# HJakeCunningham/ASVGP

Hardware: AMD Instinct MI355X
Metric: Mpoints/s per ELBO+grad step, N=10M 1D Matern-3/2 M=2048 (higher is better)
Workload: dtype f64

## Files before the change

asvgp_amd/_lib.py:

```python
import ctypes
import os

import torch

HERE = os.path.dirname(os.path.abspath(__file__))
LIB_PATH = os.path.join(HERE, "libasvgp_hip.so")

_c = ctypes
_P, _I, _L, _D, _Z = _c.c_void_p, _c.c_int, _c.c_int64, _c.c_double, _c.c_size_t

SIGNATURES = {
    "asvgp_version": (_I, []),
    "asvgp_last_error_string": (_c.c_char_p, []),
    "asvgp_status_name": (_c.c_char_p, [_I]),
    "asvgp_phi_workspace_bytes": (_Z, [_L, _I, _L]),
    "asvgp_create": (_I, [_c.POINTER(_P)]),
    "asvgp_destroy": (_I, [_P]),
    "asvgp_phi_accumulate_1d": (_I, [_P, _P, _P, _L, _L, _P, _L, _D, _I, _L, _P, _P, _Z, _P]),
    "asvgp_phi_weighted_workspace_bytes": (_Z, [_L, _I, _L]),
    "asvgp_phi_accumulate_1d_weighted": (_I, [_P, _P, _P, _P, _L, _L, _P, _L, _D, _I, _L, _P, _P, _P, _Z, _P]),
    "asvgp_set_weight_sums": (_I, [_P, _D, _D, _D]),
    "asvgp_phi_accumulate_kron2d_weighted": (_I, [_P, _P, _P, _L, _P, _L, _D, _L, _P, _L, _D, _L, _I, _P, _P, _P]),
    "asvgp_phi_accumulate_kron2d_sorted_weighted": (_I, [_P, _P, _P, _L, _P, _P, _L, _D, _L, _P, _L, _D, _L, _I, _P, _P, _P]),
    "asvgp_set_phi_algorithm": (_I, [_P, _I]),
    "asvgp_phi_last_algorithm": (_I, [_P]),
    "asvgp_set_phi_input_order": (_I, [_P, _I]),
    "asvgp_phi_last_input_order": (_I, [_P]),
    "asvgp_stream_probe": (_I, [_P, _P, _L, _P, _P]),
    "asvgp_debug_reload_env": (_I, []),
    "asvgp_set_deferred_forward_pass": (_I, [_P, _I]),
    "asvgp_prior_publish": (_I, [_P]),
    "asvgp_host_mantissa_bits": (_I, []),
    "asvgp_prior_interior_kuu_host": (_I, [_P, _I, _L, _I, _P, _P, _c.POINTER(_L), _c.POINTER(_L), _P]),
    "asvgp_result_mirror": (_I, [_P, _I, _c.POINTER(_P)]),
    "asvgp_result_mirror_read": (_I, [_P, _c.c_uint64, _P, _D]),
    "asvgp_elbo_grad_ahead_1d": (_I, [_P, _P, _P, _I, _L, _L, _I, _L, _P, _P, _P, _Z, _P]),
    "asvgp_elbo_publish_theta": (_I, [_P, _D, _D, _D]),
    "asvgp_elbo_grad_host_1d": (_I, [_P, _P, _P, _I, _D, _D, _D, _L, _L, _I, _L, _P, _P, _P, _Z, _P, _P, _D]),
    "asvgp_result_mirror_pending": (_c.c_uint64, [_P]),
    "asvgp_set_phi_workgroups": (_I, [_P, _I]),
    "asvgp_set_phi_deferred_reduce": (_I, [_P, _I]),
    "asvgp_phi_reduce_1d": (_I, [_P, _P]),
    "asvgp_phi_index_1d": (_I, [_P, _L, _P, _L, _D, _P, _P]),
    "asvgp_phi_evaluate_1d": (_I, [_P, _L, _P, _L, _D, _I, _I, _P, _P, _P]),
    "asvgp_matern_coeffs": (_I, [_I, _D, _D, _c.POINTER(_D), _c.POINTER(_D), _c.POINTER(_I)]),
    "asvgp_kuu_assemble": (_I, [_P, _I, _c.POINTER(_D), _c.POINTER(_D), _L, _I, _P, _P, _P]),
    "asvgp_cholesky_band": (_I, [_P, _P, _L, _I, _P, _P]),
    "asvgp_inverse_from_cholesky_band": (_I, [_P, _P, _L, _I, _P]),
    "asvgp_solve_triang_mat": (_I, [_P, _P, _P, _L, _I, _L, _I, _P]),
    "asvgp_product_band_band": (_I, [_P, _P, _P, _L, _I, _I, _I, _I, _I, _I, _P]),
    "asvgp_transpose_band": (_I, [_P, _P, _L, _I, _I, _P]),
    "asvgp_symmetrise_band": (_I, [_P, _P, _L, _I, _P]),
    "asvgp_unpack_banded_matrix_to_dense": (_I, [_P, _P, _L, _I, _I, _P]),
    "asvgp_pack_dense_matrix_to_banded": (_I, [_P, _P, _L, _I, _I, _P]),
    "asvgp_band_trace_sym": (_I, [_P, _P, _L, _I, _P, _P]),
    "asvgp_cholesky_band_vjp": (_I, [_P, _P, _P, _P, _L, _I, _P]),
    "asvgp_inverse_from_cholesky_band_vjp": (_I, [_P, _P, _P, _P, _P, _L, _I, _P]),
    "asvgp_band_outer_product": (_I, [_P, _P, _L, _L, _I, _D, _P, _P]),
    "asvgp_elbo_workspace_bytes": (_Z, [_L, _I, _L]),
    "asvgp_set_band_algorithm": (_I, [_P, _I]),
    "asvgp_prior_plan_1d": (_I, [_P, _P, _I, _L, _I, _c.POINTER(_I)]),
    "asvgp_prior_table_doubles": (_Z, [_P, _I, _L, _I]),
    "asvgp_prior_forward_host": (_I, [_P, _I, _L, _I, _P, _P, _P, _Z, _P]),
    "asvgp_set_prior_forward": (_I, [_P, _I]),
    "asvgp_prior_forward_device": (_I, [_P, _P, _P, _P, _Z, _P]),
# ... 109 lines not shown
        import numpy as np
        coef = np.ascontiguousarray(coef, dtype=np.float64)
        dcoef = np.ascontiguousarray(dcoef, dtype=np.float64)
        tab = np.zeros(int(n_doubles), dtype=np.float64)
        check(self._lib.asvgp_prior_forward_device(self.ptr, coef.ctypes.data, dcoef.ctypes.data, tab.ctypes.data, tab.size, stream_ptr()),
              "prior_forward_device")
        return tab

    def set_band_algorithm(self, algo):
        check(self._lib.asvgp_set_band_algorithm(self.ptr, int(algo)), "set_band_algorithm")
        self.band_algorithm = int(algo)

    def set_phi_algorithm(self, algo):
        check(self._lib.asvgp_set_phi_algorithm(self.ptr, int(algo)), "set_phi_algorithm")

    def set_weight_sums(self, n_pos, sum_w, sum_log_w):
        if n_pos is None:
            n_pos, sum_w, sum_log_w = -1.0, 0.0, 0.0
        check(self._lib.asvgp_set_weight_sums(self.ptr, float(n_pos), float(sum_w), float(sum_log_w)), "set_weight_sums")

    def phi_last_algorithm(self):
        return int(self._lib.asvgp_phi_last_algorithm(self.ptr))

    def set_phi_input_order(self, order):
        check(self._lib.asvgp_set_phi_input_order(self.ptr, int(order)), "set_phi_input_order")

    def phi_last_input_order(self):
        return int(self._lib.asvgp_phi_last_input_order(self.ptr))

    def result_mirror(self, enable=True):
        import numpy as np
        ptr = _P()
        check(self._lib.asvgp_result_mirror(self.ptr, int(bool(enable)), ctypes.byref(ptr)), "result_mirror")
        if not enable or not ptr.value:
            self._mirror = None
            return None
        self._mirror = np.ctypeslib.as_array(ctypes.cast(ptr, ctypes.POINTER(_D)), shape=(16,))
        return self._mirror

    def set_deferred_forward_pass(self, on):
        check(self._lib.asvgp_set_deferred_forward_pass(self.ptr, int(on)), "set_deferred_forward_pass")

    def publish_forward(self):
        self._lib.asvgp_prior_publish(self.ptr)

    def result_mirror_pending(self):
# ... 79 lines not shown
```

asvgp_amd/csrc/handle.hip:

```cpp
#include <sched.h>
#include <stdlib.h>
#include <string.h>
#include <time.h>

#include <condition_variable>
#include <mutex>
#include <thread>
#include <vector>

#include "handle.hpp"

namespace asvgp {

static DebugEnv g_dbg;
static std::once_flag g_dbg_once;
static void debug_env_load() {
  g_dbg.no_assembly = getenv("ASVGP_DEBUG_NO_ASSEMBLY") ? 1 : 0;
  g_dbg.chain_stamps = getenv("ASVGP_CHAIN_STAMPS") ? 1 : 0;
  g_dbg.spin_limit = getenv("ASVGP_SPIN_LIMIT") ? atol(getenv("ASVGP_SPIN_LIMIT")) : (1L << 25);
  g_dbg.host_times = getenv("ASVGP_HOST_TIMES") ? 1 : 0;
  g_dbg.plan_first = getenv("ASVGP_PLAN_FIRST") ? 1 : 0;
  g_dbg.bcr_stamps = getenv("ASVGP_BCR_STAMPS") ? atoi(getenv("ASVGP_BCR_STAMPS")) : 0;
  g_dbg.no_split = getenv("ASVGP_NO_SPLIT") ? atoi(getenv("ASVGP_NO_SPLIT")) : 0;
}
const DebugEnv& debug_env() {
  std::call_once(g_dbg_once, debug_env_load);
  return g_dbg;
}

static Handle* g_default = nullptr;
static std::mutex g_default_mu;

Handle* as_handle(asvgp_handle_t h) {
  if (h) return reinterpret_cast<Handle*>(h);
  std::lock_guard<std::mutex> lk(g_default_mu);
  if (!g_default) {
    g_default = new Handle;
    (void)hipGetDevice(&g_default->device);
  }
  return g_default;
}

static void handle_quiesce(Handle* h) {
  if (h->ahead.valid) (void)elbo_publish_theta(h, 1.0, 1.0, 1.0, true);
  handle_publish_forward(h);
  bool need_sync = false;
// ... 164 lines not shown
  return ASVGP_OK;
}

extern "C" int asvgp_create(asvgp_handle_t* out) {
  if (!out) { set_error("asvgp_create: bad argument"); return ASVGP_ERR_BAD_ARG; }
  Handle* h = new Handle;
  if (hipGetDevice(&h->device) != hipSuccess) { delete h; set_error("asvgp_create: no HIP device"); return ASVGP_ERR_HIP; }
  *out = reinterpret_cast<asvgp_handle_t>(h);
  return ASVGP_OK;
}

extern "C" int asvgp_destroy(asvgp_handle_t handle) {
  if (!handle) return ASVGP_OK;
  Handle* h = reinterpret_cast<Handle*>(handle);
  if (h->magic != 0x41535647u) { set_error("asvgp_destroy: not a handle"); return ASVGP_ERR_BAD_ARG; }
  worker_stop(h);
  plan_release(h);
  if (h->mirror_host) (void)hipHostFree(h->mirror_host);
  if (h->evK) (void)hipEventDestroy(h->evK);
  if (h->evP) (void)hipEventDestroy(h->evP);
  if (h->prof_made)
    for (int i = 0; i < PROF_RING; ++i) { (void)hipEventDestroy(h->prof_ev[i][0]); (void)hipEventDestroy(h->prof_ev[i][1]); }
  if (h->order_dev) { (void)hipFree(h->order_dev); h->order_dev = nullptr; }
  if (h->box_host) { (void)hipHostFree(h->box_host); h->box_host = nullptr; h->box_dev = nullptr; }
  h->magic = 0;
  delete h;
  return ASVGP_OK;
}

extern "C" int asvgp_set_phi_algorithm(asvgp_handle_t handle, int algo) {
  if (algo != 0 && algo != 1 && algo != 3 && algo != 5 && algo != 6) {
    set_error("set_phi_algorithm: 0 auto (6 where it applies, else 5, else 3), 1 fp64 LDS-atomic band scatter, 3 fixed-point band scatter, 5 fixed-point centred-moment scatter, 6 tile sort + register moments");
    return ASVGP_ERR_BAD_ARG;
  }
  as_handle(handle)->phi_algo = algo;
  return ASVGP_OK;
}

extern "C" int asvgp_set_phi_input_order(asvgp_handle_t handle, int order) {
  if (order < 0 || order > 2) { set_error("set_phi_input_order: 0 probe once per (x, N), 1 unsorted, 2 time series"); return ASVGP_ERR_BAD_ARG; }
  Handle* h = as_handle(handle);
  h->phi_order = order;
  h->n_order_seen = 0;
  return ASVGP_OK;
}

// ... 191 lines not shown
```

asvgp_amd/csrc/handle.hpp:

```cpp
#pragma once
#include "asvgp_common.hpp"
#include "prior_plan.hpp"

namespace asvgp {

constexpr int PROF_RING = 1024;
constexpr int TAB_SLOTS = 16;

struct Handle {
  unsigned magic = 0x41535647u;
  int device = 0;
  int phi_algo = 0, phi_blocks = 0;
  int phi_last = 0;
  bool phi_defer = false;
  struct PendingReduce { const double* partials; int G, M, K; double* stats; bool valid; const int* ranges; } pend = {nullptr, 0, 0, 0, nullptr, false, nullptr};
  int band_algo = 0;
  bool sync_on = false;
  hipEvent_t evK = nullptr, evP = nullptr;
  bool prof_on = false, prof_made = false;
  int prof_every = 1;
  long prof_calls = 0, prof_n = 0;
  hipEvent_t prof_ev[PROF_RING][2];
  PriorPlan* plan = nullptr;
  int* node_rec_dev = nullptr;
// ... 12 lines not shown
  void* worker_park = nullptr;
  int wstate = 0;
  struct PendingForward { bool valid; double coef[ASVGP_MAX_KUU_TERMS], dcoef[ASVGP_MAX_KUU_TERMS]; double* tab; int slot; unsigned long long seq; } fwd = {false, {0}, {0}, nullptr, 0, 0};
  bool prior_forward_gpu = false;
  int* dd_img_i = nullptr;
  int dd_n_img = 0;
  double* dd_img_d = nullptr;
  double* dd_tab = nullptr;
  hipStream_t dd_stream = nullptr;
  unsigned long long* dd_ready = nullptr;
  double* mirror_host = nullptr;
  double* mirror_dev = nullptr;
  unsigned long long mirror_seq = 0;
  unsigned long long mirror_pending = 0;
  struct MeshSeen { const double* ptr; long n; int regular; double step, first, last; };
  MeshSeen mesh_seen[8];
  int n_mesh_seen = 0;
  int phi_order = 0;
  struct OrderSeen { const double* ptr; long n; int series; };
  OrderSeen order_seen[8];
  int n_order_seen = 0;
  int* order_dev = nullptr;
  int phi_last_series = 0;
  bool ahead_req = false;
  void* box_host = nullptr;
  void* box_dev = nullptr;
  struct PendingAhead { bool valid; int slot; unsigned long long seq; double* tab; int kind; double N, Nw, cw; } ahead = {false, 0, 0, nullptr, 0, 0.0, 0.0, 0.0};
  bool w_set = false;
  double w_npos = 0.0, w_sum = 0.0, w_sumlog = 0.0;
};
constexpr size_t BOX_BYTES = 4096;

struct DebugEnv { int no_assembly; int chain_stamps; long spin_limit; int host_times; int plan_first; int bcr_stamps; int no_split; };
const DebugEnv& debug_env();

Handle* as_handle(asvgp_handle_t h);

bool handle_mesh_is_linspace(Handle* h, const double* mesh_dev, long n_mesh, hipStream_t st, double* step_out, double* first_out, double* last_out);

int handle_flush_phi_reduce(Handle* h, const double* stats, hipStream_t st);

void handle_publish_forward(Handle* h);
void handle_post_forward(Handle* h);

int handle_prior_dd_prepare(Handle* h);
void handle_prior_dd_release(Handle* h);
int handle_prior_dd_forward(Handle* h, const double* coef, const double* dcoef, int slot, hipStream_t st, double** tab_out, unsigned long long* stamps = nullptr,
                            unsigned long long seq = 0, const unsigned long long** ready_out = nullptr);

int elbo_publish_theta(Handle* h, double v, double l, double s, bool withdraw);

double* handle_table_acquire(Handle* h, unsigned long long* seq_out, int* slot_out);

}
```

asvgp_amd/csrc/phi_pass.hip:

```cpp
#include <stdlib.h>

#include "handle.hpp"

namespace asvgp {

constexpr int PHI_THREADS = 1024;
constexpr int PHI_CH = 32;
constexpr int PHI_MAX_BLOCKS = 256;
constexpr size_t PHI_LDS_BUDGET = 160 * 1024 - 512;

template <int K> struct FxTab {
  int g[K + 1];
  constexpr FxTab() : g{} {
    double cf[K + 1][K + 1] = {};
    for (int i = 0; i <= K; ++i)
      for (int p = 0; p <= K; ++p) cf[i][p] = piece_coef<K, 0>(i, p);
    for (int d = 0; d <= K; ++d) {
      double mx = 0.0;
      for (int i = 0; i + d <= K; ++i)
        for (int q = 0; q <= 32; ++q) {
          const double t = q / 32.0;
          double a = cf[i][K], b = cf[i + d][K];
          for (int p = K - 1; p >= 0; --p) { a = a * t + cf[i][p]; b = b * t + cf[i + d][p]; }
          if (a * b > mx) mx = a * b;
// ... 658 lines not shown
  if (lane == 0 && good) atomicAdd(count, 1);
}

static bool handle_phi_is_series(Handle* h, const double* x, long N, double m0, double inv_delta, long n_mesh, hipStream_t st) {
  if (h->phi_order == 1) return false;
  if (h->phi_order == 2) return true;
  for (int i = 0; i < h->n_order_seen; ++i)
    if (h->order_seen[i].ptr == x && h->order_seen[i].n == N) return h->order_seen[i].series != 0;
  int series = 0;
  const int nprobe = 512;
  if (N >= 128L * nprobe) {
    if (!h->order_dev && hipMalloc(&h->order_dev, sizeof(int)) != hipSuccess) h->order_dev = nullptr;
    int cnt = 0;
    if (h->order_dev && hipMemsetAsync(h->order_dev, 0, sizeof(int), st) == hipSuccess) {
      hipLaunchKernelGGL(phi_order_probe_kernel, dim3(nprobe), dim3(64), 0, st, x, N, N / nprobe, nprobe, m0, inv_delta, (int)n_mesh, h->order_dev);
      if (hipMemcpyAsync(&cnt, h->order_dev, sizeof(int), hipMemcpyDeviceToHost, st) == hipSuccess && hipStreamSynchronize(st) == hipSuccess)
        series = cnt * 10 >= nprobe * 9 ? 1 : 0;
    }
  }
  if (h->n_order_seen < 8) h->order_seen[h->n_order_seen++] = Handle::OrderSeen{x, N, series};
  return series != 0;
}

template <int K, int TP, int TS>
static int launch_phi_sort_as(Handle* h, const double* x, const double* y, long N, const double* mesh, long n_mesh, double delta,
                              long M, double* stats, double* ws, hipStream_t st, double step, double m0, double m_last, double margin) {
  size_t lds_bytes = ps_lds_bytes<K, TP, TS>();
  if (ps_epilogue_bytes<K>() > lds_bytes) lds_bytes = ps_epilogue_bytes<K>();
  if (lds_bytes > 160 * 1024) return 1;
  long nblk = (N + TP * PS_THREADS - 1) / (TP * PS_THREADS);
  const long gmax = (h->phi_blocks > 0 && h->phi_blocks < PHI_MAX_BLOCKS) ? h->phi_blocks : PHI_MAX_BLOCKS;
  const int G = (int)(nblk < 1 ? 1 : (nblk > gmax ? gmax : nblk));
  long ppb = (N + G - 1) / G;
  ppb = TS ? ((ppb + 127) & ~127L) : ((ppb + 1) & ~1L);
  if (ppb > 0x3fffffffL) return 1;
  PsArgs a;
  a.x = x; a.y = y; a.N = N; a.mesh_g = mesh; a.n_mesh = (int)n_mesh; a.inv_delta = 1.0 / delta; a.M = (int)M;
  a.m0 = m0; a.m_last = m_last; a.step = step; a.smax_fast = 0.5 - margin;
  a.partials = ws; a.ppb = ppb; a.zero_ptr = stats; a.zero_n = (K + 2) * M + 1; a.stamps = nullptr; a.stamps_wave = 0;
  a.ranges = reinterpret_cast<int*>(ws + (size_t)PHI_MAX_BLOCKS * ((size_t)(K + 2) * M + 1));
  auto kern = phi_sort_kernel<K, TP, 0, 1, TS>;
  hipError_t e = hipFuncSetAttribute(reinterpret_cast<const void*>(kern), hipFuncAttributeMaxDynamicSharedMemorySize, (int)lds_bytes);
  if (e != hipSuccess) { set_error("hipFuncSetAttribute(%zu B LDS): %s", lds_bytes, hipGetErrorString(e)); return ASVGP_ERR_LDS_CAPACITY; }
  const bool prof = h->prof_on && h->prof_n < PROF_RING && (h->prof_calls++ % h->prof_every == 0);
  if (prof) (void)hipEventRecord(h->prof_ev[h->prof_n][0], st);
  hipLaunchKernelGGL(kern, dim3((unsigned)G), dim3(PS_THREADS), lds_bytes, st, a);
  if (prof) { (void)hipEventRecord(h->prof_ev[h->prof_n][1], st); ++h->prof_n; }
  h->phi_last_series = TS;
  const int E1 = (int)((K + 2) * M + 1);
  const int gsplit = G >= 64 ? 16 : (G >= 8 ? 4 : 1);
  if (h->phi_defer) {
    h->pend = Handle::PendingReduce{a.partials, G, (int)M, K, stats, true, a.ranges};
    return check_launch("phi_accumulate_1d (tile sort, reduce deferred)");
  }
  hipLaunchKernelGGL(phi_reduce_kernel, dim3((E1 + 255) / 256, gsplit), dim3(256), 0, st, a.partials, G, (int)M, K, 0, M, 1L, 0, 1, stats, (const int*)a.ranges);
  return check_launch("phi_accumulate_1d (tile sort)");
}

template <int K>
static int launch_phi_sort(Handle* h, const double* x, const double* y, long N, long D, const double* mesh, long n_mesh, double delta,
                           long M, double* stats, double* ws, hipStream_t st) {
  if (D != 1 || N < 2 || M > PS_NCELL || ((reinterpret_cast<uintptr_t>(x) | reinterpret_cast<uintptr_t>(y)) & 15) != 0) return 1;
  double step = 0.0, m0 = 0.0, m_last = 0.0;
  if (!handle_mesh_is_linspace(h, mesh, n_mesh, st, &step, &m0, &m_last)) return 1;
  const double amax = fabs(m0) > fabs(m_last) ? fabs(m0) : fabs(m_last);
  const double margin = 16.0 * 2.220446049250313e-16 * amax / delta + 1e-12;
  if (!(margin < 0.125)) return 1;
  constexpr int TP = ps_tile_points<K>();
  constexpr int TPS = TP < 4 ? TP : 4;
  if (handle_phi_is_series(h, x, N, m0, 1.0 / delta, n_mesh, st)) {
    const int rc = launch_phi_sort_as<K, TPS, 1>(h, x, y, N, mesh, n_mesh, delta, M, stats, ws, st, step, m0, m_last, margin);
// ... 141 lines not shown
  long ppb = ((long)N + G - 1) / G;
  ppb = (ppb + 1) & ~1L;
  hipLaunchKernelGGL(stream_probe_kernel, dim3(G), dim3(1024), 0, as_stream(stream), x, y, (long)N, ppb, sink);
  return check_launch("stream_probe");
}

namespace asvgp {
int handle_flush_phi_reduce(Handle* h, const double* stats, hipStream_t st) {
  if (!h->pend.valid) return ASVGP_OK;
  if (stats && stats != h->pend.stats) return ASVGP_OK;
  const Handle::PendingReduce p = h->pend;
  h->pend.valid = false;
  const int E1 = (p.K + 2) * p.M + 1;
  const int gsplit = p.G >= 64 ? 16 : (p.G >= 8 ? 4 : 1);
  hipLaunchKernelGGL(phi_reduce_kernel, dim3((E1 + 255) / 256, gsplit), dim3(256), 0, st, p.partials, p.G, p.M, p.K, 0, (long)p.M, 1L, 0, 1, p.stats, p.ranges);
  return check_launch("phi_reduce_1d");
}
}

extern "C" int asvgp_phi_reduce_1d(asvgp_handle_t handle, asvgp_stream_t stream) {
  return handle_flush_phi_reduce(as_handle(handle), nullptr, as_stream(stream));
}

extern "C" int asvgp_phi_index_1d(const double* x, int64_t N, const double* mesh, int64_t n_mesh, double delta,
                                  int64_t* idx, asvgp_stream_t stream) {
  if (!x || !mesh || !idx || N < 0 || n_mesh < 2 || !(delta > 0.0)) { set_error("phi_index_1d: bad argument"); return ASVGP_ERR_BAD_ARG; }
  if (N == 0) return ASVGP_OK;
  hipLaunchKernelGGL(phi_index_kernel, dim3((unsigned)((N + 255) / 256)), dim3(256), 0, as_stream(stream), x, (long)N,
                     mesh, (int)n_mesh, 1.0 / delta, reinterpret_cast<long long*>(idx));
  return check_launch("phi_index_1d");
}

template <int K>
static int launch_eval(const double* x, long N, const double* mesh, int n_mesh, double delta, int deriv,
                       long long* rows, double* data, hipStream_t st) {
  dim3 g((unsigned)((N + 255) / 256)), b(256);
  double id = 1.0 / delta;
  switch (deriv) {
    case 0: hipLaunchKernelGGL((phi_evaluate_kernel<K, 0>), g, b, 0, st, x, N, mesh, n_mesh, id, rows, data); break;
    case 1: hipLaunchKernelGGL((phi_evaluate_kernel<K, (K >= 1 ? 1 : 0)>), g, b, 0, st, x, N, mesh, n_mesh, id, rows, data); break;
    case 2: hipLaunchKernelGGL((phi_evaluate_kernel<K, (K >= 2 ? 2 : 0)>), g, b, 0, st, x, N, mesh, n_mesh, id, rows, data); break;
    default: hipLaunchKernelGGL((phi_evaluate_kernel<K, (K >= 3 ? 3 : 0)>), g, b, 0, st, x, N, mesh, n_mesh, id, rows, data); break;
  }
  return check_launch("phi_evaluate_1d");
}

// ... 122 lines not shown
```

asvgp_amd/csrc/phi_sort.hpp:

```cpp
#pragma once

namespace asvgp {

constexpr int PS_THREADS = 1024;
constexpr int PS_NCELL = 2 * PS_THREADS;
constexpr int PS_HEAVY = 48;
constexpr int PS_HROUND = 16;
constexpr int PS_HLIST = 8192 / (PS_HEAVY + 1) + 1;

struct PsArgs {
  const double* x; const double* y; long N;
  const double* mesh_g; int n_mesh; double inv_delta; int M;
  double m0, m_last;
  double step;
  double smax_fast;
  double* partials;
  long ppb;
  double* zero_ptr; long zero_n;
  unsigned long long* stamps;
  int stamps_wave;
  int* ranges;
};

template <int K> constexpr int ps_tile_points() { return K <= 3 ? 8 : (K == 4 ? 6 : (K == 5 ? 4 : 2)); }
#ifndef PS_GW
#define PS_GW 4
#endif
constexpr int PS_TS_SLOTS = 256;
template <int K> constexpr size_t ps_ts_bytes() { return (size_t)PS_TS_SLOTS * (3 * K + 2) * 8 + (size_t)2 * PS_TS_SLOTS * 4; }
template <int K, int TP, int TS = 0> constexpr size_t ps_lds_bytes() {
  return (size_t)(TP * PS_THREADS + 1) * 16 + (size_t)3 * PS_NCELL * 4 + 64 * 4 + 64 * 8 +
         (size_t)PS_HROUND * (3 * K + 1) * 8 + (size_t)PS_HLIST * 12 + (TS ? ps_ts_bytes<K>() : 0);
}
template <int K> constexpr size_t ps_epilogue_bytes() {
  int all = (K + 1) * (K + 2) / 2, lo = (K + 1) + K, hi = all - lo;
  int planes = K <= 4 ? all : (lo > hi ? lo : hi);
  if (planes < 2 * (K + 1)) planes = 2 * (K + 1);
  return (size_t)planes * (PS_THREADS + K) * 8;
}

__device__ __forceinline__ void ps_lds_barrier() { asm volatile("s_waitcnt lgkmcnt(0)\n\ts_barrier" ::: "memory"); }

template <int CTRL, int ROW_MASK>
__device__ __forceinline__ unsigned ps_dpp_add_u32(unsigned v) {
  return v + (unsigned)__builtin_amdgcn_update_dpp(0, (int)v, CTRL, ROW_MASK, 0xf, true);
// ... 86 lines not shown
  for (int q = 0; q <= K; ++q) T2[q] = 0.0;
  for (unsigned sl = (unsigned)first; sl < nsl; sl += (unsigned)stride) {
    const unsigned j = sl * 64 + lane;
    if (j < hn) {
      const double2 pt = buf[ho + j];
      ps_acc<K>(pt.x, pt.y, S2, T2);
    }
  }
  if constexpr (NS <= 8) {
    int idx;
    const double t = ps_reduce_scatter8<NS>(S2, lane, idx);
    if (lane < 8 && idx < NS) lds_add(slot + idx, t);
  } else {
#pragma unroll
    for (int q = 0; q < NS; ++q) { const double t = wave_sum_dpp(S2[q]); if (lane == 0) lds_add(slot + q, t); }
  }
  __builtin_amdgcn_sched_barrier(0);
  {
    int idx;
    const double t = ps_reduce_scatter8<K + 1>(T2, lane, idx);
    if (lane < 8 && idx <= K) lds_add(slot + NS + idx, t);
  }
  __builtin_amdgcn_sched_barrier(0);
}

template <int K, int TP, int ABL = 0, int PF = 0, int TS = 0>
__global__ __launch_bounds__(PS_THREADS) void phi_sort_kernel(PsArgs a) {
  extern __shared__ double lds[];
  static_assert(TP % 2 == 0 && TP * PS_THREADS <= 8192, "tile: rank field is 13 bits");
  constexpr int T = TP * PS_THREADS;
  constexpr int NS = 2 * K;
  double2* buf = reinterpret_cast<double2*>(lds);
  unsigned* cnt = reinterpret_cast<unsigned*>(buf + T + 1);
  unsigned* off = cnt + 2 * PS_NCELL;
  unsigned* wtot = off + PS_NCELL;
  double* scratch = reinterpret_cast<double*>(wtot + 64);
  constexpr int NSTAT = 3 * K + 1;
  double* hacc = scratch + 64;
  unsigned* hlist = reinterpret_cast<unsigned*>(hacc + PS_HROUND * NSTAT);
  unsigned* nheavy_p = wtot + 32;
  constexpr int TSW = NSTAT + 1;
  double* tstab = reinterpret_cast<double*>(hlist + 3 * PS_HLIST);
  int* tskey = reinterpret_cast<int*>(tstab + PS_TS_SLOTS * TSW);
  int* tslist = tskey + PS_TS_SLOTS;
  unsigned* ts_ctl = wtot + 40;
  if (a.zero_ptr) for (long e = (long)blockIdx.x * blockDim.x + threadIdx.x; e < a.zero_n; e += (long)gridDim.x * blockDim.x) a.zero_ptr[e] = 0.0;
// ... 472 lines not shown
  if (a.ranges) {
    const unsigned mn = n0A ? (unsigned)tid : (n0B ? (unsigned)(tid + PS_THREADS) : 0x7fffffu);
    const unsigned mx = n0B ? (unsigned)(tid + PS_THREADS) + 1u : (n0A ? (unsigned)tid + 1u : 0u);
    const unsigned wmn = ps_wave_min_u32(mn), wmx = ps_wave_max_u32(mx);
    if (lane == 0) { wtot[wv] = wmn; wtot[16 + wv] = wmx; }
    __syncthreads();
    const unsigned bmn = ps_wave_min_u32(wtot[lane & 15]), bmx = ps_wave_max_u32(wtot[16 + (lane & 15)]);
    col_lo = bmx ? (int)bmn : 1;
    col_hi = bmx ? (int)bmx - 1 + K : 0;
    if (col_hi > M - 1) col_hi = M - 1;
    if (tid == 0) { a.ranges[2 * blockIdx.x] = col_lo; a.ranges[2 * blockIdx.x + 1] = col_hi; }
    __syncthreads();
  }
  if constexpr (ABL == 5) {
    double keep = (double)(n0A + n0B);
#pragma unroll
    for (int p = 0; p < NS; ++p) keep += SA[p] + SB[p];
#pragma unroll
    for (int p = 0; p <= K; ++p) keep += TA[p] + TB[p];
    out[tid] = keep;
  } else if constexpr (ABL == 0 || ABL == 9) {
    constexpr int IW = PS_THREADS + K;
    double* img = lds;
    auto q_planes = [&](const double (&S)[NS], unsigned n0, int slot, int d0, int d1) __attribute__((always_inline)) {
      const double s0v = (double)n0;
      int pid = 0;
      if (!__any(n0 != 0u)) {
#pragma unroll
        for (int d = d0; d < d1; ++d)
#pragma unroll
          for (int i = 0; i + d <= K; ++i) img[(pid++) * IW + slot] = 0.0;
        return;
      }
#pragma unroll
      for (int d = d0; d < d1; ++d) {
#pragma unroll
        for (int i = 0; i + d <= K; ++i) {
          const int j = i + d, mi = K - j, mj = K - i;
          if (mi < i) continue;
          double e = MomCoef<K>::tab.pair[i][j][0] * s0v, o = 0.0;
#pragma unroll
          for (int p = 2; p <= NS; p += 2) e = fma(MomCoef<K>::tab.pair[i][j][p], S[p - 1], e);
          if (mi != i) {
#pragma unroll
            for (int p = 1; p <= NS; p += 2) o = fma(MomCoef<K>::tab.pair[i][j][p], S[p - 1], o);
            img[(pid + mi) * IW + slot] = e - o;
// ... 24 lines not shown
#pragma unroll
      for (int rnd = 0; rnd < (DSPLIT <= K ? 2 : 1); ++rnd) {
        const int d0 = rnd == 0 ? 0 : DSPLIT, d1 = rnd == 0 ? DSPLIT : K + 1;
        if (half == 0) q_planes(SA, n0A, K + tid, d0, d1); else q_planes(SB, n0B, K + tid, d0, d1);
        if (tid >= PS_THREADS - K) {
          const int hs = tid - (PS_THREADS - K);
          if (half == 0) {
            int np = 0;
#pragma unroll
            for (int d = d0; d < d1; ++d) np += K + 1 - d;
            for (int pl = 0; pl < np; ++pl) img[pl * IW + hs] = 0.0;
          } else {
            q_planes(SA, n0A, hs, d0, d1);
          }
        }
        ps_lds_barrier();
        if (j < M && j >= col_lo && j <= col_hi) {
          int pid = 0;
#pragma unroll
          for (int d = d0; d < d1; ++d) {
            double v = 0.0;
#pragma unroll
            for (int jj = d; jj <= K; ++jj) v += img[(pid + jj - d) * IW + tid + jj];
            __builtin_nontemporal_store((j + d < M) ? v : 0.0, out + (size_t)d * M + j);
            pid += K + 1 - d;
          }
        }
        ps_lds_barrier();
      }
    }
    r_planes(TA, K + tid, 0);
    r_planes(TB, K + tid, K + 1);
    if (tid >= PS_THREADS - K) {
      const int hs = tid - (PS_THREADS - K);
#pragma unroll
      for (int i = 0; i <= K; ++i) img[i * IW + hs] = 0.0;
      r_planes(TA, hs, K + 1);
    }
    ps_lds_barrier();
#pragma unroll
    for (int half = 0; half < 2; ++half) {
      const int j = half * PS_THREADS + tid;
      if (j < M && j >= col_lo && j <= col_hi) {
        double r = 0.0;
#pragma unroll
        for (int i = 0; i <= K; ++i) r += img[(half * (K + 1) + i) * IW + tid + i];
        __builtin_nontemporal_store(r, out + (size_t)(K + 1) * M + j);
      }
    }
    if (tid == 0) out[(size_t)(K + 2) * M] = (badf > 0.0) ? __builtin_nan("") : tot;
  } else {
    if (tid == 0) out[0] = tot + badf;
  }
  stamp(4);
  if constexpr (ABL == 9) {
    if (tid == (int)(a.stamps_wave * 64) && a.stamps)
      for (int i = 0; i < 8; ++i) a.stamps[(size_t)blockIdx.x * 8 + i] = ph[i];
  }
}

}
```

include/asvgp_hip.h:

```cpp
#ifndef ASVGP_HIP_H
#define ASVGP_HIP_H

#include <stddef.h>
#include <stdint.h>

#ifdef __cplusplus
extern "C" {
#endif

typedef void* asvgp_stream_t;
typedef struct asvgp_handle_s* asvgp_handle_t;

typedef enum {
  ASVGP_OK = 0,
  ASVGP_ERR_BAD_ARG = -1,
  ASVGP_ERR_UNSUPPORTED = -2,
  ASVGP_ERR_LDS_CAPACITY = -3,
  ASVGP_ERR_WORKSPACE = -4,
  ASVGP_ERR_HIP = -5
} asvgp_status;

enum { ASVGP_MATERN12 = 0, ASVGP_MATERN32 = 1, ASVGP_MATERN52 = 2 };
enum { ASVGP_MAX_ORDER = 6, ASVGP_MAX_BANDWIDTH = 8, ASVGP_MAX_KUU_TERMS = 9 };

// ... 13 lines not shown
int asvgp_prior_interior_kuu_host(const double* static_bands_host, int n_terms, int64_t M, int k, const double* coef_host,
                                  double* kuu_diag8, int64_t* lo, int64_t* hi, double* bnd256);
int asvgp_host_mantissa_bits(void);
int asvgp_debug_reload_env(void);
int asvgp_set_deferred_forward_pass(asvgp_handle_t handle, int on);
int asvgp_prior_publish(asvgp_handle_t handle);
int asvgp_result_mirror(asvgp_handle_t handle, int enable, const double** host_ptr);
uint64_t asvgp_result_mirror_pending(asvgp_handle_t handle);
int asvgp_result_mirror_read(asvgp_handle_t handle, uint64_t token, double* result10, double timeout_seconds);
int asvgp_elbo_grad_ahead_1d(asvgp_handle_t handle, const double* stats, const double* static_bands, int kind, int64_t N, int64_t M, int k,
                             int64_t D, double* out, int* info, void* workspace, size_t workspace_bytes, asvgp_stream_t stream);
int asvgp_elbo_publish_theta(asvgp_handle_t handle, double variance, double lengthscale, double noise_variance);
int asvgp_elbo_grad_host_1d(asvgp_handle_t handle, const double* stats, const double* static_bands, int kind, double variance,
                            double lengthscale, double noise_variance, int64_t N, int64_t M, int k, int64_t D,
                            double* out, int* info, void* workspace, size_t workspace_bytes, asvgp_stream_t stream,
                            double* result10, double timeout_seconds);
int asvgp_phi_last_algorithm(asvgp_handle_t handle);
int asvgp_set_phi_input_order(asvgp_handle_t handle, int order);
int asvgp_phi_last_input_order(asvgp_handle_t handle);
int asvgp_stream_probe(const double* x, const double* y, int64_t N, double* sink, asvgp_stream_t stream);
int asvgp_set_phi_workgroups(asvgp_handle_t handle, int n);
int asvgp_set_phi_deferred_reduce(asvgp_handle_t handle, int on);
int asvgp_phi_reduce_1d(asvgp_handle_t handle, asvgp_stream_t stream);

size_t asvgp_phi_weighted_workspace_bytes(int64_t M, int order, int64_t D);
int asvgp_phi_accumulate_1d_weighted(asvgp_handle_t handle, const double* x, const double* y, const double* w, int64_t N, int64_t D,
                                     const double* mesh, int64_t n_mesh, double delta, int order, int64_t M, double* stats,
                                     double* wstats, void* workspace, size_t workspace_bytes, asvgp_stream_t stream);
int asvgp_set_weight_sums(asvgp_handle_t handle, double n_pos, double sum_w, double sum_log_w);

int asvgp_phi_index_1d(const double* x, int64_t N, const double* mesh, int64_t n_mesh, double delta,
                       int64_t* idx, asvgp_stream_t stream);

int asvgp_phi_evaluate_1d(const double* x, int64_t N, const double* mesh, int64_t n_mesh, double delta,
                          int order, int deriv, int64_t* rows, double* data, asvgp_stream_t stream);

int asvgp_matern_coeffs(int kind, double variance, double lengthscale, double* coef_host, double* dcoef_dl_host,
                        int* n_terms_host);
int asvgp_kuu_assemble(const double* static_bands, int n_terms, const double* coef_host,
                       const double* dcoef_dl_host, int64_t M, int k, double* Kuu, double* dKuu_dl,
                       asvgp_stream_t stream);

int asvgp_cholesky_band(const double* K, double* L, int64_t M, int k, int* info, asvgp_stream_t stream);
int asvgp_inverse_from_cholesky_band(const double* L, double* S, int64_t M, int k, asvgp_stream_t stream);
int asvgp_solve_triang_mat(const double* L, const double* B, double* X, int64_t M, int k, int64_t D,
                           int transpose_left, asvgp_stream_t stream);
// ... 175 lines not shown
```

Before: 135,700.

## Fuse cross-block partial reduction into phi sort kernel tail with work stealing

Replaces the separate reduction launch after the tile-sort phi kernel. Blocks now finish the cross-workgroup sum of partial statistics inside the same kernel, using an arrival counter, a bounded spin and a last-block sweep that steals slices nobody claimed. Partials are written with agent-scope atomic stores so other blocks see them. It also caches the LDS attribute call so it is not repeated on every launch. The cost is spin-waiting and atomic-store overhead, and correctness now relies on a rotating set of device-resident control slots.

```diff
diff --git a/asvgp_amd/_lib.py b/asvgp_amd/_lib.py
--- a/asvgp_amd/_lib.py
+++ b/asvgp_amd/_lib.py
@@ -41,6 +41,8 @@
     "asvgp_set_phi_workgroups": (_I, [_P, _I]),
     "asvgp_set_phi_deferred_reduce": (_I, [_P, _I]),
     "asvgp_phi_reduce_1d": (_I, [_P, _P]),
+    "asvgp_phi_last_tail_sum": (_I, [_P]),
+    "asvgp_phi_tail_diag": (_I, [_P, _c.POINTER(_c.c_uint32), _I]),
     "asvgp_phi_index_1d": (_I, [_P, _L, _P, _L, _D, _P, _P]),
     "asvgp_phi_evaluate_1d": (_I, [_P, _L, _P, _L, _D, _I, _I, _P, _P, _P]),
     "asvgp_matern_coeffs": (_I, [_I, _D, _D, _c.POINTER(_D), _c.POINTER(_D), _c.POINTER(_I)]),
@@ -196,6 +198,14 @@
     def phi_last_algorithm(self):
         return int(self._lib.asvgp_phi_last_algorithm(self.ptr))
 
+    def phi_last_tail_sum(self):
+        return int(self._lib.asvgp_phi_last_tail_sum(self.ptr))
+
+    def phi_tail_diag(self, reset=True):
+        out = (_c.c_uint32 * 4)()
+        check(self._lib.asvgp_phi_tail_diag(self.ptr, out, int(bool(reset))), "phi_tail_diag")
+        return {"max_wait_us": out[0] / 100.0, "expired": int(out[1]), "swept": int(out[2]), "launches": int(out[3])}
+
     def set_phi_input_order(self, order):
         check(self._lib.asvgp_set_phi_input_order(self.ptr, int(order)), "set_phi_input_order")
 
diff --git a/asvgp_amd/csrc/handle.hip b/asvgp_amd/csrc/handle.hip
--- a/asvgp_amd/csrc/handle.hip
+++ b/asvgp_amd/csrc/handle.hip
@@ -22,6 +22,9 @@
   g_dbg.plan_first = getenv("ASVGP_PLAN_FIRST") ? 1 : 0;
   g_dbg.bcr_stamps = getenv("ASVGP_BCR_STAMPS") ? atoi(getenv("ASVGP_BCR_STAMPS")) : 0;
   g_dbg.no_split = getenv("ASVGP_NO_SPLIT") ? atoi(getenv("ASVGP_NO_SPLIT")) : 0;
+  g_dbg.phi_tail = getenv("ASVGP_PHI_TAIL_REDUCE") ? atoi(getenv("ASVGP_PHI_TAIL_REDUCE")) : 1;
+  g_dbg.phi_tail_spin_us = getenv("ASVGP_PHI_TAIL_SPIN") ? atol(getenv("ASVGP_PHI_TAIL_SPIN")) : PHI_TAIL_WAIT_US;
+  g_dbg.phi_tail_diag = getenv("ASVGP_PHI_TAIL_DIAG") ? 1 : 0;
 }
 const DebugEnv& debug_env() {
   std::call_once(g_dbg_once, debug_env_load);
@@ -232,6 +235,7 @@
   if (h->prof_made)
     for (int i = 0; i < PROF_RING; ++i) { (void)hipEventDestroy(h->prof_ev[i][0]); (void)hipEventDestroy(h->prof_ev[i][1]); }
   if (h->order_dev) { (void)hipFree(h->order_dev); h->order_dev = nullptr; }
+  if (h->phi_tail_dev) { (void)hipFree(h->phi_tail_dev); h->phi_tail_dev = nullptr; }
   if (h->box_host) { (void)hipHostFree(h->box_host); h->box_host = nullptr; h->box_dev = nullptr; }
   h->magic = 0;
   delete h;
diff --git a/asvgp_amd/csrc/handle.hpp b/asvgp_amd/csrc/handle.hpp
--- a/asvgp_amd/csrc/handle.hpp
+++ b/asvgp_amd/csrc/handle.hpp
@@ -58,6 +58,9 @@
   int n_order_seen = 0;
   int* order_dev = nullptr;
   int phi_last_series = 0;
+  unsigned* phi_tail_dev = nullptr;
+  unsigned long long phi_tail_seq = 0;
+  int phi_last_tail = 0;
   bool ahead_req = false;
   void* box_host = nullptr;
   void* box_dev = nullptr;
@@ -66,8 +69,13 @@
   double w_npos = 0.0, w_sum = 0.0, w_sumlog = 0.0;
 };
 constexpr size_t BOX_BYTES = 4096;
+constexpr int PHI_TAIL_SLOTS = 8;
+constexpr int PHI_TAIL_WORDS = 512;
+constexpr int PHI_TAIL_STATE0 = 32;
+constexpr int PHI_TAIL_DIAG = 4;
+constexpr long PHI_TAIL_WAIT_US = 2000;
 
-struct DebugEnv { int no_assembly; int chain_stamps; long spin_limit; int host_times; int plan_first; int bcr_stamps; int no_split; };
+struct DebugEnv { int no_assembly; int chain_stamps; long spin_limit; int host_times; int plan_first; int bcr_stamps; int no_split; int phi_tail; long phi_tail_spin_us; int phi_tail_diag; };
 const DebugEnv& debug_env();
 
 Handle* as_handle(asvgp_handle_t h);
diff --git a/asvgp_amd/csrc/phi_pass.hip b/asvgp_amd/csrc/phi_pass.hip
--- a/asvgp_amd/csrc/phi_pass.hip
+++ b/asvgp_amd/csrc/phi_pass.hip
@@ -704,9 +704,22 @@
   return series != 0;
 }
 
+static int handle_phi_tail_prepare(Handle* h, hipStream_t st) {
+  if (h->phi_tail_dev) return ASVGP_OK;
+  const size_t bytes = sizeof(unsigned) * ((size_t)PHI_TAIL_SLOTS * PHI_TAIL_WORDS + PHI_TAIL_DIAG);
+  unsigned* p = nullptr;
+  hipError_t e = hipMalloc(&p, bytes);
+  if (e == hipSuccess) e = hipMemsetAsync(p, 0, bytes, st);
+  if (e == hipSuccess) e = hipStreamSynchronize(st);
+  if (e != hipSuccess) { if (p) (void)hipFree(p); set_error("phi_accumulate_1d: control blocks of the tail sum: %s", hipGetErrorString(e)); return ASVGP_ERR_HIP; }
+  h->phi_tail_dev = p;
+  return ASVGP_OK;
+}
+
 template <int K, int TP, int TS>
 static int launch_phi_sort_as(Handle* h, const double* x, const double* y, long N, const double* mesh, long n_mesh, double delta,
                               long M, double* stats, double* ws, hipStream_t st, double step, double m0, double m_last, double margin) {
+  static_assert(PHI_TAIL_WORDS == PS_TAIL_WORDS && PHI_TAIL_STATE0 == PS_TAIL_STATE0 && PS_TAIL_STATE0 + PHI_MAX_BLOCKS <= PS_TAIL_WORDS, "control block layout");
   size_t lds_bytes = ps_lds_bytes<K, TP, TS>();
   if (ps_epilogue_bytes<K>() > lds_bytes) lds_bytes = ps_epilogue_bytes<K>();
   if (lds_bytes > 160 * 1024) return 1;
@@ -716,19 +729,45 @@
   long ppb = (N + G - 1) / G;
   ppb = TS ? ((ppb + 127) & ~127L) : ((ppb + 1) & ~1L);
   if (ppb > 0x3fffffffL) return 1;
+  const DebugEnv& dbg = debug_env();
+  const bool tail = TS == 0 && dbg.phi_tail != 0;
   PsArgs a;
   a.x = x; a.y = y; a.N = N; a.mesh_g = mesh; a.n_mesh = (int)n_mesh; a.inv_delta = 1.0 / delta; a.M = (int)M;
   a.m0 = m0; a.m_last = m_last; a.step = step; a.smax_fast = 0.5 - margin;
   a.partials = ws; a.ppb = ppb; a.zero_ptr = stats; a.zero_n = (K + 2) * M + 1; a.stamps = nullptr; a.stamps_wave = 0;
   a.ranges = reinterpret_cast<int*>(ws + (size_t)PHI_MAX_BLOCKS * ((size_t)(K + 2) * M + 1));
+  a.tail = nullptr; a.tail_clean = nullptr; a.tail_stats = nullptr; a.tail_ticks = 0; a.tail_diag = nullptr;
+  if (tail) {
+    a.zero_ptr = nullptr; a.zero_n = 0;
+    a.ranges = nullptr;
+    if (G == 1) {
+      a.partials = stats;
+    } else {
+      const int rc = handle_phi_tail_prepare(h, st);
+      if (rc) return rc;
+      const unsigned long long n = h->phi_tail_seq++;
+      a.tail = h->phi_tail_dev + (size_t)(n % PHI_TAIL_SLOTS) * PHI_TAIL_WORDS;
+      a.tail_clean = h->phi_tail_dev + (size_t)((n + PHI_TAIL_SLOTS / 2) % PHI_TAIL_SLOTS) * PHI_TAIL_WORDS;
+      a.tail_stats = stats;
+      a.tail_ticks = dbg.phi_tail_spin_us > 0 ? dbg.phi_tail_spin_us * 100 : 0;
+      a.tail_diag = dbg.phi_tail_diag ? h->phi_tail_dev + (size_t)PHI_TAIL_SLOTS * PHI_TAIL_WORDS : nullptr;
+    }
+  }
   auto kern = phi_sort_kernel<K, TP, 0, 1, TS>;
-  hipError_t e = hipFuncSetAttribute(reinterpret_cast<const void*>(kern), hipFuncAttributeMaxDynamicSharedMemorySize, (int)lds_bytes);
-  if (e != hipSuccess) { set_error("hipFuncSetAttribute(%zu B LDS): %s", lds_bytes, hipGetErrorString(e)); return ASVGP_ERR_LDS_CAPACITY; }
+  static size_t lds_granted[16] = {0};
+  size_t& granted = lds_granted[h->device & 15];
+  if (lds_bytes > granted) {
+    hipError_t e = hipFuncSetAttribute(reinterpret_cast<const void*>(kern), hipFuncAttributeMaxDynamicSharedMemorySize, (int)lds_bytes);
+    if (e != hipSuccess) { set_error("hipFuncSetAttribute(%zu B LDS): %s", lds_bytes, hipGetErrorString(e)); return ASVGP_ERR_LDS_CAPACITY; }
+    granted = lds_bytes;
+  }
   const bool prof = h->prof_on && h->prof_n < PROF_RING && (h->prof_calls++ % h->prof_every == 0);
   if (prof) (void)hipEventRecord(h->prof_ev[h->prof_n][0], st);
   hipLaunchKernelGGL(kern, dim3((unsigned)G), dim3(PS_THREADS), lds_bytes, st, a);
   if (prof) { (void)hipEventRecord(h->prof_ev[h->prof_n][1], st); ++h->prof_n; }
   h->phi_last_series = TS;
+  h->phi_last_tail = tail ? 1 : 0;
+  if (tail) return check_launch("phi_accumulate_1d (tile sort, tail sum)");
   const int E1 = (int)((K + 2) * M + 1);
   const int gsplit = G >= 64 ? 16 : (G >= 8 ? 4 : 1);
   if (h->phi_defer) {
@@ -916,6 +955,19 @@
   return handle_flush_phi_reduce(as_handle(handle), nullptr, as_stream(stream));
 }
 
+extern "C" int asvgp_phi_tail_diag(asvgp_handle_t handle, uint32_t* out4, int reset) {
+  Handle* h = as_handle(handle);
+  if (!out4) { set_error("phi_tail_diag: bad argument"); return ASVGP_ERR_BAD_ARG; }
+  out4[0] = out4[1] = out4[2] = out4[3] = 0;
+  if (!h->phi_tail_dev) return ASVGP_OK;
+  unsigned* d = h->phi_tail_dev + (size_t)PHI_TAIL_SLOTS * PHI_TAIL_WORDS;
+  if (hipDeviceSynchronize() != hipSuccess || hipMemcpy(out4, d, sizeof(unsigned) * PHI_TAIL_DIAG, hipMemcpyDeviceToHost) != hipSuccess ||
+      (reset && hipMemset(d, 0, sizeof(unsigned) * PHI_TAIL_DIAG) != hipSuccess)) { set_error("phi_tail_diag: copy failed"); return ASVGP_ERR_HIP; }
+  return ASVGP_OK;
+}
+
+extern "C" int asvgp_phi_last_tail_sum(asvgp_handle_t handle) { return as_handle(handle)->phi_last_tail; }
+
 extern "C" int asvgp_phi_index_1d(const double* x, int64_t N, const double* mesh, int64_t n_mesh, double delta,
                                   int64_t* idx, asvgp_stream_t stream) {
   if (!x || !mesh || !idx || N < 0 || n_mesh < 2 || !(delta > 0.0)) { set_error("phi_index_1d: bad argument"); return ASVGP_ERR_BAD_ARG; }
diff --git a/asvgp_amd/csrc/phi_sort.hpp b/asvgp_amd/csrc/phi_sort.hpp
--- a/asvgp_amd/csrc/phi_sort.hpp
+++ b/asvgp_amd/csrc/phi_sort.hpp
@@ -20,7 +20,10 @@
   unsigned long long* stamps;
   int stamps_wave;
   int* ranges;
+  unsigned* tail = nullptr; unsigned* tail_clean = nullptr; double* tail_stats = nullptr; long tail_ticks = 0; unsigned* tail_diag = nullptr;
 };
+constexpr int PS_TAIL_STATE0 = 32;
+constexpr int PS_TAIL_WORDS = 512;
 
 template <int K> constexpr int ps_tile_points() { return K <= 3 ? 8 : (K == 4 ? 6 : (K == 5 ? 4 : 2)); }
 #ifndef PS_GW
@@ -153,6 +156,100 @@
     if (lane < 8 && idx <= K) lds_add(slot + NS + idx, t);
   }
   __builtin_amdgcn_sched_barrier(0);
+}
+
+__device__ __forceinline__ void ps_tail_sum_slice(const double* partials, int G, int E1, int per, int sl, double* stats, double* red, int tid) {
+  const int e0 = sl * per;
+  int e1 = e0 + per;
+  if (e1 > E1) e1 = E1;
+  if (e0 >= e1) return;
+  const int rsplit = G >= 16 ? 16 : (G >= 8 ? 8 : (G >= 4 ? 4 : (G >= 2 ? 2 : 1))), csplit = 16 / rsplit;
+  const int lane = tid & 63, w = tid >> 6, rgrp = w & (rsplit - 1), cgrp = w / rsplit;
+  const int nch = (e1 - e0 + 63) >> 6, iters = (nch + csplit - 1) / csplit;
+  for (int it = 0; it < iters; ++it) {
+    const int c = it * csplit + cgrp, e = e0 + (c << 6) + lane;
+    const bool valid = c < nch && e < e1;
+    const double* col = partials + (valid ? e : e0);
+    double v[16];
+#pragma unroll
+    for (int j = 0; j < 16; ++j) {
+      const int row = rgrp + j * rsplit;
+      v[j] = col[(size_t)(row < G ? row : G - 1) * (size_t)E1];
+    }
+    double acc[4] = {0.0, 0.0, 0.0, 0.0};
+#pragma unroll
+    for (int j = 0; j < 16; ++j) acc[j & 3] += (rgrp + j * rsplit < G) ? v[j] : 0.0;
+    red[w * 64 + lane] = (acc[0] + acc[1]) + (acc[2] + acc[3]);
+    __syncthreads();
+    if (rgrp == 0 && valid) {
+      double t = 0.0;
+      for (int r = 0; r < rsplit; ++r) t += red[(cgrp * rsplit + r) * 64 + lane];
+      stats[e] = t;
+    }
+    __syncthreads();
+  }
+}
+
+__device__ __forceinline__ void ps_tail_sum(const PsArgs& a, int E1, double* red, unsigned* ctl, int tid) {
+  const int G = (int)gridDim.x, g = (int)blockIdx.x;
+  const int per = (E1 + G - 1) / G;
+  unsigned* ctr = a.tail;
+  unsigned* state = a.tail + PS_TAIL_STATE0;
+  if (g == 0 && a.tail_clean)
+    for (int i = tid; i < PS_TAIL_WORDS; i += PS_THREADS) __hip_atomic_store(a.tail_clean + i, 0u, __ATOMIC_RELAXED, __HIP_MEMORY_SCOPE_AGENT);
+  asm volatile("s_waitcnt vmcnt(0)" ::: "memory");
+  __syncthreads();
+  if (tid == 0) {
+    __builtin_amdgcn_fence(__ATOMIC_RELEASE, "agent");
+    asm volatile("s_waitcnt vmcnt(0)" ::: "memory");
+    const unsigned prev = __hip_atomic_fetch_add(ctr, 1u, __ATOMIC_RELAXED, __HIP_MEMORY_SCOPE_AGENT);
+    const bool last = prev == (unsigned)(G - 1);
+    bool ready = last;
+    if (!last && a.tail_ticks > 0) {
+      const unsigned long long t0 = __builtin_amdgcn_s_memrealtime();
+      unsigned long long waited = 0;
+      for (;;) {
+        if (__hip_atomic_load(ctr, __ATOMIC_RELAXED, __HIP_MEMORY_SCOPE_AGENT) >= (unsigned)G) { ready = true; break; }
+        waited = __builtin_amdgcn_s_memrealtime() - t0;
+        if (waited > (unsigned long long)a.tail_ticks) break;
+        __builtin_amdgcn_s_sleep(4);
+      }
+      if (a.tail_diag) {
+        waited = __builtin_amdgcn_s_memrealtime() - t0;
+        __hip_atomic_fetch_max(a.tail_diag, (unsigned)(waited > 0xffffffffull ? 0xffffffffull : waited), __ATOMIC_RELAXED, __HIP_MEMORY_SCOPE_AGENT);
+        if (!ready) __hip_atomic_fetch_add(a.tail_diag + 1, 1u, __ATOMIC_RELAXED, __HIP_MEMORY_SCOPE_AGENT);
+      }
+    }
+    bool mine = false;
+    if (ready) {
+      unsigned expect = 0u;
+      mine = __hip_atomic_compare_exchange_strong(state + g, &expect, 1u, __ATOMIC_RELAXED, __ATOMIC_RELAXED, __HIP_MEMORY_SCOPE_AGENT);
+      __builtin_amdgcn_fence(__ATOMIC_ACQUIRE, "agent");
+    }
+    ctl[0] = mine ? 1u : 0u;
+    ctl[1] = last ? 1u : 0u;
+    if (last && a.tail_diag) __hip_atomic_fetch_add(a.tail_diag + 3, 1u, __ATOMIC_RELAXED, __HIP_MEMORY_SCOPE_AGENT);
+  }
+  asm volatile("s_waitcnt vmcnt(0)" ::: "memory");
+  __syncthreads();
+  const bool mine = ctl[0] != 0u, last = ctl[1] != 0u;
+  if (mine) ps_tail_sum_slice(a.partials, G, E1, per, g, a.tail_stats, red, tid);
+  if (!last) return;
+  __syncthreads();
+  unsigned* list = ctl + 2;
+  if (tid == 0) list[0] = 0u;
+  __syncthreads();
+  if (tid < G && tid != g && __hip_atomic_load(state + tid, __ATOMIC_RELAXED, __HIP_MEMORY_SCOPE_AGENT) == 0u) {
+    unsigned expect = 0u;
+    if (__hip_atomic_compare_exchange_strong(state + tid, &expect, 1u, __ATOMIC_RELAXED, __ATOMIC_RELAXED, __HIP_MEMORY_SCOPE_AGENT)) {
+      const unsigned pos = __hip_atomic_fetch_add(list, 1u, __ATOMIC_RELAXED, __HIP_MEMORY_SCOPE_WORKGROUP);
+      list[1 + pos] = (unsigned)tid;
+    }
+  }
+  __syncthreads();
+  const unsigned nsw = list[0];
+  for (unsigned i = 0; i < nsw; ++i) ps_tail_sum_slice(a.partials, G, E1, per, (int)list[1 + i], a.tail_stats, red, tid);
+  if (tid == 0 && a.tail_diag && nsw) __hip_atomic_fetch_add(a.tail_diag + 2, nsw, __ATOMIC_RELAXED, __HIP_MEMORY_SCOPE_AGENT);
 }
 
 template <int K, int TP, int ABL = 0, int PF = 0, int TS = 0>
@@ -671,6 +768,10 @@
   } else if constexpr (ABL == 0 || ABL == 9) {
     constexpr int IW = PS_THREADS + K;
     double* img = lds;
+    const bool tailsum = TS == 0 && a.tail != nullptr;
+    auto pstore = [&](double v, double* p) __attribute__((always_inline)) {
+      if (tailsum) __hip_atomic_store(p, v, __ATOMIC_RELAXED, __HIP_MEMORY_SCOPE_AGENT); else __builtin_nontemporal_store(v, p);
+    };
     auto q_planes = [&](const double (&S)[NS], unsigned n0, int slot, int d0, int d1) __attribute__((always_inline)) {
       const double s0v = (double)n0;
       int pid = 0;
@@ -741,7 +842,7 @@
             double v = 0.0;
 #pragma unroll
             for (int jj = d; jj <= K; ++jj) v += img[(pid + jj - d) * IW + tid + jj];
-            __builtin_nontemporal_store((j + d < M) ? v : 0.0, out + (size_t)d * M + j);
+            pstore((j + d < M) ? v : 0.0, out + (size_t)d * M + j);
             pid += K + 1 - d;
           }
         }
@@ -764,10 +865,17 @@
         double r = 0.0;
 #pragma unroll
         for (int i = 0; i <= K; ++i) r += img[(half * (K + 1) + i) * IW + tid + i];
-        __builtin_nontemporal_store(r, out + (size_t)(K + 1) * M + j);
-      }
-    }
-    if (tid == 0) out[(size_t)(K + 2) * M] = (badf > 0.0) ? __builtin_nan("") : tot;
+        pstore(r, out + (size_t)(K + 1) * M + j);
+      }
+    }
+    if (tid == 0) pstore((badf > 0.0) ? __builtin_nan("") : tot, out + (size_t)(K + 2) * M);
+    if constexpr (TS == 0) {
+      if (tailsum) {
+        stamp(4);
+        ps_tail_sum(a, (K + 2) * M + 1, lds, wtot, tid);
+        stamp(-1);
+      }
+    }
   } else {
     if (tid == 0) out[0] = tot + badf;
   }
diff --git a/include/asvgp_hip.h b/include/asvgp_hip.h
--- a/include/asvgp_hip.h
+++ b/include/asvgp_hip.h
@@ -59,6 +59,8 @@
 int asvgp_set_phi_workgroups(asvgp_handle_t handle, int n);
 int asvgp_set_phi_deferred_reduce(asvgp_handle_t handle, int on);
 int asvgp_phi_reduce_1d(asvgp_handle_t handle, asvgp_stream_t stream);
+int asvgp_phi_last_tail_sum(asvgp_handle_t handle);
+int asvgp_phi_tail_diag(asvgp_handle_t handle, uint32_t* out4, int reset);
 
 size_t asvgp_phi_weighted_workspace_bytes(int64_t M, int order, int64_t D);
 int asvgp_phi_accumulate_1d_weighted(asvgp_handle_t handle, const double* x, const double* y, const double* w, int64_t N, int64_t D,
```

Result: slower. 111,300 (-18.0%).
